# google/balloon-learning-environment

Hardware: AMD Instinct MI355X
Metric: env-steps/sec at 65 536 parallel envs; achieved HBM GB/s fraction of peak (higher is better)
Workload: dtype f32+f64

## Files before the change

balloon_learning_environment_amd/csrc/ble_step_core.h:

```cpp
#pragma once
#include "ble_physics.h"

namespace ble {

struct StateDev {
  float *x, *y, *pressure, *ambient_temperature, *internal_temperature, *envelope_volume, *superpressure, *mols_air, *battery_charge;
  float *acs_power, *acs_mass_flow, *solar_charging, *power_load;
  const float *center_lat_deg, *center_lng_deg, *upwelling_infrared, *alpha;
  const int64_t* start_unix;
  int32_t *time_elapsed_s, *sunrise_h_rel, *sunset_rel;
  uint8_t *status, *last_command, *alt_fsm, *env_fsm, *power_paused;
  double* episode_cache;
};
struct EnvRegs {
  float x, y, p, t_amb, t_int, vol, sp, n_air, batt;
  float acs_power, mdot, charge, load;
  int32_t t_elapsed, sunrise_h, sunset;
  uint8_t status, alt_fsm, env_fsm, paused;
};
struct EnvConst {
  float lat0_deg, lng0_deg, ir, alpha;
  int64_t start_unix;
};
struct EnvHoisted {
  AtmBase atm;
  double sin_lat0, cos_lat0;
  double q_earth;
  uint32_t flags;
};
constexpr int kEpisodeCacheRows = 7;
BLE_FN EnvHoisted hoist_constants(const EnvConst& c) {
  EnvHoisted h;
  h.atm = atm_base((double)c.alpha);
  sincos_f64((double)c.lat0_deg * (kPiD / 180.0), &h.sin_lat0, &h.cos_lat0);
  h.flags = 0;
  h.q_earth = earth_heat_per_area_f64((double)c.ir, &h.flags);
  return h;
}
BLE_FN uint32_t float_bits(float v) { uint32_t u; __builtin_memcpy(&u, &v, 4); return u; }
BLE_FN void episode_cache_keys(const EnvConst& c, uint64_t* k1, uint64_t* k2) {
  *k1 = ((uint64_t)float_bits(c.alpha) << 32) | (uint64_t)float_bits(c.lat0_deg);
  *k2 = ((uint64_t)float_bits(c.ir) << 32) | 0x80000000ull;
}
BLE_FN void episode_cache_store(double* cache, int64_t n, int64_t i, const EnvConst& c, const EnvHoisted& h) {
  uint64_t k1, k2;
  episode_cache_keys(c, &k1, &k2);
  k2 |= (uint64_t)(h.flags & 0x7fffffffu);
  double d1, d2;
  __builtin_memcpy(&d1, &k1, 8); __builtin_memcpy(&d2, &k2, 8);
  cache[i] = h.atm.p1; cache[n + i] = h.atm.p2; cache[2 * n + i] = h.sin_lat0; cache[3 * n + i] = h.cos_lat0;
  cache[4 * n + i] = h.q_earth; cache[5 * n + i] = d1; cache[6 * n + i] = d2;
}
struct EpisodeCacheRow { double v[kEpisodeCacheRows]; };
BLE_FN EpisodeCacheRow episode_cache_load(const double* cache, int64_t n, int64_t i) {
  EpisodeCacheRow r;
#pragma unroll
  for (int k = 0; k < kEpisodeCacheRows; ++k) r.v[k] = cache[k * n + i];
  return r;
}
BLE_FN bool episode_cache_hit(const EpisodeCacheRow& r, const EnvConst& c) {
  uint64_t k1, k2, g1, g2;
  episode_cache_keys(c, &k1, &k2);
  __builtin_memcpy(&g1, &r.v[5], 8); __builtin_memcpy(&g2, &r.v[6], 8);
  return g1 == k1 && (g2 & 0xffffffff80000000ull) == k2;
}
BLE_FN EnvHoisted hoisted_from_cache(const EpisodeCacheRow& r, const EnvConst& c) {
  EnvHoisted h;
  atm_base_linear((double)c.alpha, &h.atm);
  h.atm.p1 = r.v[0]; h.atm.p2 = r.v[1];
  h.sin_lat0 = r.v[2]; h.cos_lat0 = r.v[3]; h.q_earth = r.v[4];
  uint64_t g2;
  __builtin_memcpy(&g2, &r.v[6], 8);
  h.flags = (uint32_t)(g2 & 0x7fffffffull);
  return h;
}


BLE_FN double inv_cbrt_volume(double vol) {
  double yc = (double)f_exp2((-1.0f / 3.0f) * f_log2((float)vol));
  return yc * d_fma(-vol * yc, yc * yc, 4.0) * (1.0 / 3.0);
}
BLE_FN double d_min_raw(double a, double b) {
#if defined(__HIP_DEVICE_COMPILE__)
  double r; asm("v_min_f64 %0, %1, %2" : "=v"(r) : "v"(a), "v"(b)); return r;
#else
  return d_min(a, b);
#endif
}
BLE_FN double d_max_raw(double a, double b) {
#if defined(__HIP_DEVICE_COMPILE__)
  double r; asm("v_max_f64 %0, %1, %2" : "=v"(r) : "v"(a), "v"(b)); return r;
#else
  return d_max(a, b);
#endif
}
struct LayerCursor {
  int lay;
  double lapse_cur;
  double kl_cur;
  double cur_hi, cur_lo;
};
BLE_FN double stride_pressure(const AtmWindow& win, const LayerCursor& lc, double p, double rp, double vol, double n_air,
                              double t_amb, double t_at_p, double yc, const StrideK& K, double drag_arg = VehicleDefault::drag_arg) {
  const double mass = d_fma(kAirMolarMassD, n_air, K.dry_mass);
  const double num = d_fma(p * vol, K.m_over_r, -mass * t_amb);
  const double dir = __builtin_copysign(1.0, num);
  const double arg = drag_arg * __builtin_fabs(num) * rp * (yc * yc);
  const double rate = atm_rate_over_delta_height_f64(win, lc.lay, lc.lapse_cur, lc.kl_cur, lc.cur_hi, lc.cur_lo, p, rp, dir, t_at_p,
                                                     d_max(arg, 1e-30), K);
  return d_fma(rate, K.ten, p);
}
BLE_FN double stride_internal_temperature(double vol, double yc, double t_int, double t_amb, double p, float flux, float att,
                                          double q_earth, const StrideK& K, double thermal_scale = VehicleDefault::thermal_scale) {
  return t_int + thermal_increment_f64(vol, yc, t_int, t_amb, p, (double)((flux * att) * (0.25f * kSolarAbsorptivityTotal)), q_earth, K, thermal_scale);
}
template <bool kNodeFromTable = true>
BLE_FN void stride_acs(const double* acs_poly, int eff, double sp, double p, double rp, double t_int, float* acs_w, double* mdot_d,
                       const StrideK& K, double valve_k = VehicleDefault::valve_k) {
  const double a2 = d_max((2.0 * (kAirMolarMassD / kGasConstantD)) * (sp * (sp + p)), 1e-30);
  const double mdot_up = (valve_k * a2) * d_rsqrt(a2 * t_int);
  const double prm1 = d_max(sp * rp, 0.0);
  double w_down, mdot_down;
  acs_down_poly<kNodeFromTable>(acs_poly, prm1, &w_down, &mdot_down, K);
  *acs_w = eff == kDown ? (float)w_down : 0.0f;
  *mdot_d = eff == kUp ? mdot_up : (eff == kDown ? mdot_down : 0.0);
}
BLE_FN double stride_mols_air(double n_air, double mdot_d) {
  return d_max(d_fma(mdot_d, 10.0 / kAirMolarMassD, n_air), 0.0);
}
BLE_FN void stride_power_from_factor(bool is_day, float panel_factor, float att, float acs_w, float* charge, float* load, float* batt,
                                     float day_load = VehicleDefault::day_load, float night_load = VehicleDefault::night_load,
                                     float capacity = VehicleDefault::capacity) {
  *charge = is_day ? solar_power_from_factor(panel_factor, att) : 0.0f;
  *load = (is_day ? day_load : night_load) + acs_w;
  *batt = f_clamp(f_fma(*charge - *load, kStride / 3600.0f, *batt), 0.0f, capacity);
}
BLE_FN void stride_power(const SunState& sun, float att, float acs_w, float* charge, float* load, float* batt,
                         float day_load = VehicleDefault::day_load, float night_load = VehicleDefault::night_load,
                         float capacity = VehicleDefault::capacity) {
  stride_power_from_factor(sun.day, solar_panel_factor(sun), att, acs_w, charge, load, batt, day_load, night_load, capacity);
}
BLE_FN double stride_ambient_advance(const AtmWindow& win, LayerCursor& lc, double p, double rp, double t_at_p, double p_new,
                                     const StrideK& K) {
  const double kInf = (double)__builtin_huge_valf();
  double anchor_p = p, anchor_rp = rp, anchor_t = t_at_p;
  const bool crossed = p_new > lc.cur_hi || !(p_new > lc.cur_lo);
  if (__builtin_expect(wave_any(crossed), 0)) if (crossed) {
    BLE_STEP_EVENT(1);
    const int lay_new = atm_window_layer(win, p_new);
    const bool low_pair = (lc.lay + lay_new) < 0;
    anchor_p = low_pair ? win.pb : win.pt;
    anchor_rp = low_pair ? win.r_pb : win.r_pt;
    anchor_t = low_pair ? win.tb : win.tt;
    lc.lay = lay_new;
    lc.lapse_cur = pick3(lay_new, win.lapse_m1, win.lapse_0, win.lapse_p1);
    lc.kl_cur = (-kAirSpecificGasD / 9.80665) * lc.lapse_cur;
    lc.cur_hi = lay_new < 0 ? kInf : (lay_new == 0 ? win.pb : win.pt);
    lc.cur_lo = lay_new < 0 ? win.pb : (lay_new == 0 ? win.pt : -kInf);
  }
  return atm_temperature_advance(anchor_t, anchor_p, anchor_rp, p_new, lc.kl_cur, K);
}

struct SolarNodes {
  double sb0, cb0, sb1, cb1, sb2, cb2;
  double sd0, cd0, hsd, hcd;
};
BLE_FN SolarNodes solar_nodes_time(const Ephemeris& e0, int64_t t0, float lng0_deg, float step_s) {
  SolarNodes n;
  double sod;
  if (__builtin_expect(t0 >= 0 && t0 < 4294967296LL, 1)) sod = (double)((uint32_t)t0 % 86400u);
  else { int64_t m = t0 % 86400; sod = (double)(m < 0 ? m + 86400 : m); }
  const double b0 = sod * (1.0 / 240.0) + 0.25 * e0.eot_min + (double)lng0_deg;
  const double half_db = 0.5 * ((double)step_s * (1.0 / 240.0) + 0.25 * (double)(e0.eot_min_rate * step_s));
  double sb0, cb0;
  sincos_f64(b0 * (kPiD / 180.0), &sb0, &cb0);
  const double hr = half_db * (kPiD / 180.0), h2 = hr * hr;
  const double sh = hr * d_fma(h2, d_fma(h2, d_fma(h2, -1.0 / 5040.0, 1.0 / 120.0), -1.0 / 6.0), 1.0);
  const double ch = d_fma(h2, d_fma(h2, d_fma(h2, -1.0 / 720.0, 1.0 / 24.0), -0.5), 1.0);
  const double sb1 = sb0 * ch + cb0 * sh, cb1 = cb0 * ch - sb0 * sh;
  const double sb2 = sb1 * ch + cb1 * sh, cb2 = cb1 * ch - sb1 * sh;
  n.sb0 = sb0; n.cb0 = cb0; n.sb1 = sb1; n.cb1 = cb1; n.sb2 = sb2; n.cb2 = cb2;
  const double sd0 = (double)e0.sin_decl, cd0 = d_sqrt_fast(d_fma(-sd0, sd0, 1.0));
  const double hsd = 0.5 * (double)(e0.sin_decl_rate * step_s), hcd = -(sd0 * d_rcp(cd0)) * hsd;
  n.sd0 = sd0; n.cd0 = cd0; n.hsd = hsd; n.hcd = hcd;
  return n;
}
template <int j>
BLE_FN double solar_node(const SolarNodes& n, double sl0, double cl0, float x_m, float y_m, float u, float v, int substeps) {
  const double x0 = (double)x_m, y0 = (double)y_m;
  const double dx = (double)u * (5.0 * (double)substeps), dy = (double)v * (5.0 * (double)substeps);
  if (j == 0) return sun_one_minus_sin_f64(sl0, cl0, x0, y0, n.sb0, n.cb0, n.sd0, n.cd0);
  if (j == 1) return sun_one_minus_sin_f64(sl0, cl0, x0 + dx, y0 + dy, n.sb1, n.cb1, n.sd0 + n.hsd, n.cd0 + n.hcd);
  return sun_one_minus_sin_f64(sl0, cl0, x0 + 2.0 * dx, y0 + 2.0 * dy, n.sb2, n.cb2, n.sd0 + 2.0 * n.hsd, n.cd0 + 2.0 * n.hcd);
}
struct SunQuadratic { float c0, c1, c2; SunThresholds thr; };
BLE_FN SunQuadratic solar_node_coefs(double f0, double f1, double f2, int substeps) {
  const double inv_2m = d_rcp((double)substeps);
  SunQuadratic sq;
  sq.c0 = (float)f0;
  sq.c1 = (float)((-f2 + 4.0 * f1 - 3.0 * f0) * inv_2m);
  sq.c2 = (float)((f2 - 2.0 * f1 + f0) * (2.0 * (inv_2m * inv_2m)));
  sq.thr = sun_thresholds(f0, substeps);
  return sq;
}
BLE_FN SunQuadratic solar_nodes_site(const SolarNodes& n, double sl0, double cl0, float x_m, float y_m, float u, float v, int substeps) {
  const double f0 = solar_node<0>(n, sl0, cl0, x_m, y_m, u, v, substeps);
  const double f1 = solar_node<1>(n, sl0, cl0, x_m, y_m, u, v, substeps);
  const double f2 = solar_node<2>(n, sl0, cl0, x_m, y_m, u, v, substeps);
  return solar_node_coefs(f0, f1, f2, substeps);
}
BLE_FN SunState sun_at_stride(int kk, const SunQuadratic& sq, const EnvConst& c, float u, float v, float x_start,
                              float y_start, int32_t t_start) {
  const float fkk = (float)kk;
  bool near;
  const float q = fkk * f_fma(fkk, sq.c2, sq.c1);
  SunState r = sun_fast(sq.c0 + q, q, sq.thr, &near);
  if (__builtin_expect(wave_any(near), 0)) if (near) {
    BLE_STEP_EVENT(0);
    kk = i_opaque(kk);
    const double dk = 10.0 * (double)kk;
    r = sun_exact((double)c.lat0_deg, (double)c.lng0_deg, d_fma(dk, (double)u, (double)x_start), d_fma(dk, (double)v, (double)y_start),
                  c.start_unix + (int64_t)(t_start + 10 * kk));
  }
  return r;
}
BLE_FN bool battery_above_99_percent(float batt, double capacity_wh = VehicleDefault::capacity_d) {
  return capacity_wh == 3058.56 ? batt >= 3027.9746f : (double)batt / capacity_wh > 0.99;
}
template <typename PowerFn>
BLE_FN float step_reward_from_power(int action, float x, float y, float batt, float acs_power, PowerFn power_end,
                                    float day_load = VehicleDefault::day_load, double capacity_wh = VehicleDefault::capacity_d) {
  float r = reward_distance(x, y);
  if (action == kDown) {
    const float pw = power_end();
    const bool excess = (pw > day_load) && battery_above_99_percent(batt, capacity_wh);
    if (!excess) {
      const float scale = f_clamp((acs_power - 100.0f) * (1.0f / 200.0f), 0.0f, 1.0f);
      r *= f_fma(-0.3f, scale, 0.95f);
    }
  }
  return r;
}
template <typename SunFn>
BLE_FN float step_reward(int action, float x, float y, float p, float batt, float acs_power, SunFn sun_end,
                         float day_load = VehicleDefault::day_load, double capacity_wh = VehicleDefault::capacity_d) {
  return step_reward_from_power(action, x, y, batt, acs_power, [&]() {
    const SunState sun = sun_end();
    return solar_power(sun, solar_attenuation(sun.sin_el, p, sun.day));
  }, day_load, capacity_wh);
}

constexpr int kTermSaveRows = 14, kTermSaveStride = 64;
constexpr int kTermAbsBit = 1 << 16;
struct NoHelper { static constexpr bool kOn = false; };
struct SunRecord { float diff, panel_factor, flux; uint32_t bits; };
template <class V = VehicleDefault, class H = NoHelper>
BLE_FN int agent_step(EnvRegs& s, const EnvConst& c, const EnvHoisted& hc, int action, const WindCorners& corners, const WindQuery& wq,
                      float noise_u, float noise_v, int substeps, const double* acs_poly, const StrideK& K, float* term_save,
                      float* reward, uint32_t* flags, const V& veh = V(), H* helper = nullptr) {
  BLE_STEP_TICK(0);
  float u, v;
  if constexpr (H::kOn) {
    wind_blend_corners(corners, wq, &u, &v);
    u += noise_u; v += noise_v;
    helper->publish(s.x, s.y, u, v, s.t_elapsed);
  }
  const float p0_in = s.p;
  double p = (double)s.p;
  const AtmWindow win = atm_window_from(hc.atm, (double)c.alpha, p, flags);
  double altitude, t_at_p;
  atm_at_pressure_f64(win, (double)c.alpha, p, &altitude, &t_at_p);
  LayerCursor lc;
  lc.lay = 0; lc.lapse_cur = win.lapse_0; lc.kl_cur = (-kAirSpecificGasD / 9.80665) * win.lapse_0; lc.cur_hi = win.pb; lc.cur_lo = win.pt;

  int eff = action;
  if (veh.power_layer)
    eff = power_safety(action, s.t_elapsed, s.batt, &s.sunrise_h, &s.sunset, &s.paused, veh.night_load_d, veh.capacity_d);
  eff = envelope_safety(eff, s.sp, &s.env_fsm, veh.max_sp);
  eff = altitude_safety(eff, altitude, &s.alt_fsm);
  BLE_STEP_TICK(1);

  const int64_t t0 = c.start_unix + (int64_t)s.t_elapsed;
  const Ephemeris e0 = ephemeris(t0);
  const float step_s = (float)(10 * substeps);
  const float fl0 = e0.flux, dfl = e0.flux_rate * 10.0f;
  BLE_STEP_TICK(2);
  if constexpr (!H::kOn) {
    wind_blend_corners(corners, wq, &u, &v);
    u += noise_u; v += noise_v;
  }
  BLE_STEP_TICK(3);
  const SolarNodes nodes = solar_nodes_time(e0, t0, c.lng0_deg, step_s);
  const SunQuadratic sq = solar_nodes_site(nodes, hc.sin_lat0, hc.cos_lat0, s.x, s.y, u, v, substeps);
  BLE_STEP_TICK(4);
  const float x_start = s.x, y_start = s.y;
  const int32_t t_start = s.t_elapsed;
  auto sun_at = [&](int kk) -> SunState {
    return sun_at_stride(kk, sq, c, u, v, x_start, y_start, t_start);
  };
  const double q_earth = hc.q_earth;
  *flags |= hc.flags;

  double t_amb = (double)s.t_amb, t_int = (double)s.t_int, n_air = (double)s.n_air, vol = (double)s.vol,
         sp = (double)s.sp;
  double t_int_lo = t_int, t_int_hi = t_int;
  float x = s.x, y = s.y, batt = s.batt;
  float acs_w = s.acs_power, charge = s.charge, load = s.load;
  double mdot_d = (double)s.mdot;
  int status = kOk;

  float* const term_word = term_save + (kTermSaveRows - 1) * kTermSaveStride;
  *term_word = 0.0f;
  auto stride = [&](const int k) __attribute__((always_inline)) {
    const float pf = (float)p;
    const double rp = d_rcp(p);
    t_int_lo = d_min_raw(t_int_lo, t_int); t_int_hi = d_max_raw(t_int_hi, t_int);
    SunState sun;
    SunRecord rec;
    float flux;
    if constexpr (!H::kOn) {
      const float fk = (float)k;
      sun = sun_at(k);
      flux = f_fma(fk, dfl, fl0);
    } else {
      rec = helper->record(k);
      flux = rec.flux;
    }

    const double yc = inv_cbrt_volume(vol);
    const double p_new = stride_pressure(win, lc, p, rp, vol, n_air, t_amb, t_at_p, yc, K, veh.drag_arg);

    float att;
    if constexpr (!H::kOn) att = solar_attenuation(sun.sin_el, pf, sun.day);
    else att = solar_attenuation_from_diff(rec.diff, pf, (rec.bits & 1u) != 0);
    const double t_int_new = stride_internal_temperature(vol, yc, t_int, t_amb, p, flux, att, q_earth, K, veh.thermal_scale);

    double vol_new, sp_new;
    superpressure_volume_f64(n_air, t_int, p, rp, &vol_new, &sp_new, K, veh.dvdp, veh.four_dvdp, veh.inv_dvdp);
    bool terminal = !(sp_new <= veh.max_sp) || sp_new <= 0.0;

    stride_acs(acs_poly, eff, sp, p, rp, t_int, &acs_w, &mdot_d, K, veh.valve_k);
    const double n_air_new = stride_mols_air(n_air, mdot_d);

    if constexpr (!H::kOn) stride_power(sun, att, acs_w, &charge, &load, &batt, veh.day_load, veh.night_load, veh.capacity);
    else stride_power_from_factor((rec.bits & 1u) != 0, rec.panel_factor, att, acs_w, &charge, &load, &batt, veh.day_load, veh.night_load, veh.capacity);
    terminal = terminal || batt <= 0.0f;

    x = f_fma(u, kStride, x);
    y = f_fma(v, kStride, y);
    t_amb = t_at_p;
    t_at_p = stride_ambient_advance(win, lc, p, rp, t_at_p, p_new, K);
    p = p_new; t_int = t_int_new; vol = vol_new; sp = sp_new; n_air = n_air_new;
    if (__builtin_expect(wave_any(terminal), 0)) if (terminal && __builtin_bit_cast(int, *term_word) == 0) {
      int st = kOk;
      if (!(sp <= veh.max_sp)) st = kBurst;
      if (sp <= 0.0) st = kZeroPressure;
      if (batt <= 0.0f) st = kOutOfPower;
      const float parked[kTermSaveRows - 1] = {x, y, (float)p, (float)t_amb, (float)t_int, (float)vol, (float)sp, (float)n_air, batt,
                                               acs_w, (float)mdot_d, charge, load};
#pragma unroll
      for (int j = 0; j < kTermSaveRows - 1; ++j) term_save[j * kTermSaveStride] = parked[j];
      const int strides = i_opaque(k + 1);
      const int abs_bad = absorptivity_out_of_range(t_int_lo) || absorptivity_out_of_range(t_int_hi) ? kTermAbsBit : 0;
      *term_word = __builtin_bit_cast(float, st | (strides << 8) | abs_bad);
      if constexpr (H::kOn) helper->park_reward_record(k + 1);
    }
  };
  int ks = 0;
#pragma unroll 1
  for (; ks + 1 < substeps; ks += 2) { stride(ks); stride(ks + 1); }
  if (ks < substeps) stride(ks);
  BLE_STEP_TICK(5);
  s.x = x; s.y = y; s.p = (float)p; s.t_amb = (float)t_amb; s.t_int = (float)t_int; s.vol = (float)vol;
  s.sp = (float)sp; s.n_air = (float)n_air; s.batt = batt;
  s.acs_power = acs_w; s.mdot = (float)mdot_d; s.charge = charge; s.load = load;
  int k = substeps;
  const int word = __builtin_bit_cast(int, *term_word);
  const bool done = word != 0;
  SunRecord rec_end;
  if constexpr (H::kOn) rec_end = helper->record_end(substeps);
  bool abs_bad = absorptivity_out_of_range(t_int_lo) || absorptivity_out_of_range(t_int_hi);
  if (__builtin_expect(wave_any(done), 0)) if (done) {
    s.x = term_save[0]; s.y = term_save[kTermSaveStride]; s.p = term_save[2 * kTermSaveStride]; s.t_amb = term_save[3 * kTermSaveStride];
    s.t_int = term_save[4 * kTermSaveStride]; s.vol = term_save[5 * kTermSaveStride]; s.sp = term_save[6 * kTermSaveStride];
    s.n_air = term_save[7 * kTermSaveStride]; s.batt = term_save[8 * kTermSaveStride]; s.acs_power = term_save[9 * kTermSaveStride];
    s.mdot = term_save[10 * kTermSaveStride]; s.charge = term_save[11 * kTermSaveStride]; s.load = term_save[12 * kTermSaveStride];
    status = word & 0xff; k = (word >> 8) & 0xff; abs_bad = (word & kTermAbsBit) != 0;
    if constexpr (H::kOn) rec_end = helper->parked_reward_record();
  }
  s.t_elapsed += 10 * k;
  s.status = (uint8_t)status;
  *flags |= abs_bad ? kFlagAbsorptivity : 0u;

  *flags |= (s.p > 101325.0f || s.p < 0.0f || p0_in > 101325.0f || p0_in < 0.0f) ? kFlagSolarRange : 0u;

  if constexpr (!H::kOn) {
  *reward = step_reward(action, s.x, s.y, s.p, s.batt, s.acs_power, [&]() { return sun_at(k); }, veh.day_load, veh.capacity_d);
  } else {
    *reward = step_reward_from_power(action, s.x, s.y, s.batt, s.acs_power, [&]() {
      return solar_power_from_factor(rec_end.panel_factor, solar_attenuation_from_diff(rec_end.diff, s.p, (rec_end.bits & 1u) != 0));
    }, veh.day_load, veh.capacity_d);
  }
  BLE_STEP_TICK(6);
  return eff;
}

}
```

balloon_learning_environment_amd/csrc/ble_step_helper.h:

```cpp
#pragma once
#include "ble_step_core.h"

namespace ble {

constexpr int kHelperGroups = 4;
constexpr int kHelperBlock = 2 * 64 * kHelperGroups;
constexpr int kHelperRing = 32;

struct alignas(16) HelperGroupShared {
  SunRecord ring[kHelperRing][64];
  SunRecord reward_park[64];
  float x[64], y[64], u[64], v[64];
  int32_t t_elapsed[64];
  unsigned long long live;
  int steps_published;
  int records_taken;
  int records_ready;
  int pad_;
};
struct HelperShared {
  HelperGroupShared group[kHelperGroups];
  int ticket[4];
  int placed[kHelperBlock / 64];
};

BLE_FN int helper_uniform(int v) { return __builtin_amdgcn_readfirstlane(v); }
BLE_FN int helper_counter_load(const int* p) { return helper_uniform(__hip_atomic_load(p, __ATOMIC_RELAXED, __HIP_MEMORY_SCOPE_WORKGROUP)); }
BLE_FN void helper_counter_store(int* p, int v) {
  asm volatile("s_waitcnt lgkmcnt(0)" ::: "memory");
  __hip_atomic_store(p, v, __ATOMIC_RELAXED, __HIP_MEMORY_SCOPE_WORKGROUP);
}
BLE_FN void helper_wait_above(const int* p, int need, int* seen) {
  int r = helper_counter_load(p);
  while (r <= need) { __builtin_amdgcn_s_sleep(1); r = helper_counter_load(p); }
  *seen = r;
  asm volatile("" ::: "memory");
}

BLE_FN int helper_assign_roles(HelperShared& sh, int hw_wave, int lane) {
  const int simd = (int)__builtin_amdgcn_s_getreg((1 << 11) | (4 << 6) | 4) & 3;
  const int tid = hw_wave * 64 + lane;
  if (tid < 4) sh.ticket[tid] = 0;
  if (tid < kHelperGroups) {
    sh.group[tid].live = 0ull; sh.group[tid].steps_published = 0; sh.group[tid].records_taken = 0; sh.group[tid].records_ready = 0;
  }
  __syncthreads();
  if (lane == 0) {
    const int t = atomicAdd(&sh.ticket[simd], 1);
    sh.placed[hw_wave] = t < 2 ? 2 * simd + t : -1;
  }
  __syncthreads();
  constexpr int kWaves = kHelperBlock / 64;
  int taken = 0, unplaced_before = 0;
#pragma unroll
  for (int q = 0; q < kWaves; ++q) {
    const int p = helper_uniform(sh.placed[q]);
    if (p >= 0) taken |= 1 << p;
    else if (q < hw_wave) ++unplaced_before;
  }
  int role = helper_uniform(sh.placed[hw_wave]);
  if (role < 0) {
    role = 0;
#pragma unroll
    for (int r = 0, free_seen = 0; r < kWaves; ++r)
      if (!((taken >> r) & 1)) { if (free_seen == unplaced_before) role = r; ++free_seen; }
  }
  return role;
}

struct HelperMain {
  static constexpr bool kOn = true;
  HelperGroupShared* g;
  int lane;
  int base, ready_seen, steps_done;
  BLE_FN void publish(float x, float y, float u, float v, int32_t t_elapsed) {
    g->x[lane] = x; g->y[lane] = y; g->u[lane] = u; g->v[lane] = v; g->t_elapsed[lane] = t_elapsed;
    g->live = __builtin_amdgcn_ballot_w64(true);
    helper_counter_store(&g->steps_published, steps_done);
  }
  BLE_FN SunRecord read(int index) const { return g->ring[index & (kHelperRing - 1)][lane]; }
  BLE_FN SunRecord record(int k) {
    const int index = helper_uniform(base) + k;
    if ((k & 1) == 0) {
      asm volatile("" ::: "memory");
      __hip_atomic_store(&g->records_taken, index, __ATOMIC_RELAXED, __HIP_MEMORY_SCOPE_WORKGROUP);
    }
    if (__builtin_expect(helper_uniform(ready_seen) <= index, 0)) helper_wait_above(&g->records_ready, index, &ready_seen);
    return read(index);
  }
  BLE_FN SunRecord record_end(int substeps) {
    const int index = helper_uniform(base) + substeps;
    if (__builtin_expect(helper_uniform(ready_seen) <= index, 0)) helper_wait_above(&g->records_ready, index, &ready_seen);
    const SunRecord r = read(index);
    base = index + 1;
    return r;
  }
  BLE_FN void park_reward_record(int k) {
    const int index = helper_uniform(base) + k;
    int seen;
    helper_wait_above(&g->records_ready, index, &seen);
    g->reward_park[lane] = read(index);
  }
  BLE_FN SunRecord parked_reward_record() const { return g->reward_park[lane]; }
  BLE_FN void publish_idle() {
    g->live = 0ull;
    helper_counter_store(&g->steps_published, steps_done);
  }
};

BLE_FN void helper_wave(const StateDev& st, HelperGroupShared* g, int lane, int64_t i, bool in_range, int substeps, int n_steps) {
  EnvConst c = {0.0f, 0.0f, 0.0f, 0.0f, 0};
  int32_t t_s = 0;
  bool ok = false;
  if (in_range) {
    c.lat0_deg = st.center_lat_deg[i]; c.lng0_deg = st.center_lng_deg[i];
    c.ir = st.upwelling_infrared[i]; c.alpha = st.alpha[i]; c.start_unix = st.start_unix[i];
    t_s = st.time_elapsed_s[i];
    ok = st.status[i] == kOk;
  }
  double sin_lat0 = 0.0, cos_lat0 = 1.0;
  if (ok) sincos_f64((double)c.lat0_deg * (kPiD / 180.0), &sin_lat0, &cos_lat0);
  const float step_s = (float)(10 * substeps);
  int next = 0;
  int taken_seen = 0, published_seen = 0;
  bool all_frozen = false;
#pragma unroll 1
  for (int step = 0; step < n_steps; ++step) {
    int64_t t0 = c.start_unix + (int64_t)t_s;
    Ephemeris e0 = {};
    SolarNodes nodes = {};
    if (!all_frozen) {
      e0 = ephemeris(t0);
      nodes = solar_nodes_time(e0, t0, c.lng0_deg, step_s);
    }
    if (published_seen <= step) helper_wait_above(&g->steps_published, step, &published_seen);
    const unsigned long long live_mask = g->live;
    const uint32_t live_lo = (uint32_t)helper_uniform((int)(uint32_t)live_mask), live_hi = (uint32_t)helper_uniform((int)(uint32_t)(live_mask >> 32));
    if (live_lo == 0u && live_hi == 0u) { all_frozen = true; continue; }
    const bool live = (((lane < 32 ? live_lo : live_hi) >> (lane & 31)) & 1u) != 0u;
    float x = g->x[lane], y = g->y[lane], u = g->u[lane], v = g->v[lane];
    int32_t t_pub = g->t_elapsed[lane];
    if (!live) { x = 0.0f; y = 0.0f; u = 0.0f; v = 0.0f; t_pub = t_s; }
    const bool moved = t_pub != t_s;
    if (__builtin_expect(wave_any(moved), 0)) if (moved) {
      t_s = t_pub;
      t0 = c.start_unix + (int64_t)t_s;
      e0 = ephemeris(t0);
      nodes = solar_nodes_time(e0, t0, c.lng0_deg, step_s);
    }
    const float fl0 = e0.flux, dfl = e0.flux_rate * 10.0f;
    const SunQuadratic sq = solar_nodes_site(nodes, sin_lat0, cos_lat0, x, y, u, v, substeps);
#pragma unroll 1
    for (int kk = 0; kk <= substeps; ++kk) {
      const SunState sun = sun_at_stride(kk, sq, c, u, v, x, y, t_s);
      SunRecord rec;
      rec.diff = solar_airmass_diff(sun.sin_el);
      rec.panel_factor = solar_panel_factor(sun);
      rec.flux = f_fma((float)kk, dfl, fl0);
      rec.bits = sun.day ? 1u : 0u;
      if (__builtin_expect(next - taken_seen >= kHelperRing, 0)) helper_wait_above(&g->records_taken, next - kHelperRing, &taken_seen);
      g->ring[next & (kHelperRing - 1)][lane] = rec;
      ++next;
      helper_counter_store(&g->records_ready, next);
    }
    t_s += 10 * substeps;
  }
}

}
```

profiles/isa_histogram.py:

```python
import os
import re
import subprocess
import sys
import tempfile

sys.path.insert(0, os.path.dirname(os.path.abspath(__file__)))
from isa_compare import ROOT, assemble

DEFAULT_KERNEL = 'ble_step_kernelILb0EN3ble14VehicleDefaultEEE'
CLASSES = ['fp64 arithmetic', 'fp32 arithmetic', 'v_cmp*', 'v_cndmask*', 'v_cvt*', 'other vector', 'moves', 'LDS', 'memory', 'SALU',
           'branches', 'waits', 's_nop']


def classify(op: str) -> str:
  if op.startswith('v_cmp'):
    return 'v_cmp*'
  if op.startswith('v_cndmask'):
    return 'v_cndmask*'
  if op.startswith('v_cvt'):
    return 'v_cvt*'
  if op.startswith(('v_mov', 'v_accvgpr', 'v_readfirstlane', 'v_readlane', 'v_writelane', 'v_swap')):
    return 'moves'
  if op.startswith('v_'):
    if '_f64' in op:
      return 'fp64 arithmetic'
    if '_f32' in op or '_f16' in op:
      return 'fp32 arithmetic'
    return 'other vector'
  if op.startswith('ds_'):
    return 'LDS'
  if op.startswith(('global_', 'buffer_', 'flat_', 'scratch_', 's_load', 's_buffer_load')):
    return 'memory'
  if op.startswith('s_waitcnt') or op.startswith('s_wait'):
    return 'waits'
  if op == 's_nop':
    return 's_nop'
  if op.startswith(('s_cbranch', 's_branch')):
    return 'branches'
  return 'SALU'


def kernel_body(asm: str, key: str):
  lines = asm.splitlines()
  start = next(i for i, l in enumerate(lines) if re.match(r'^\S*' + re.escape(key) + r'\S*:', l))
  out, parents, loop = [], {}, None
  for i in range(start + 1, len(lines)):
    if re.match(r'^\.Lfunc_end\d+:', lines[i]):
      break
    text, _, comment = lines[i].partition(';')
    text = text.strip()
    label = re.match(r'^(\.LBB\d+_\d+):', text)
    if label or re.match(r'^\s*; %bb\.\d+:', lines[i]):
      block_comment = lines[i]
      for j in range(i + 1, min(i + 4, len(lines))):
        if not lines[j].lstrip().startswith(';') or '%bb.' in lines[j]:
          break
        block_comment += lines[j]
      m = re.search(r'in Loop: Header=(BB\d+_\d+)', block_comment)
      if m:
        loop = '.L' + m.group(1)
      elif 'Loop Header' in block_comment and label:
        loop = label.group(1)
        m = re.findall(r'Parent Loop (BB\d+_\d+)', block_comment)
        parents[loop] = '.L' + m[-1] if m else None
      else:
        loop = None
    if text and (label or not text.startswith('.')):
      out.append((i + 1, text, loop))
  return lines[start].split(':')[0], out, parents


def in_loop(loop, header, parents) -> bool:
  while loop is not None:
    if loop == header:
      return True
    loop = parents.get(loop)
  return False


def hot_path(body, parents, header, inner=None):
  label_at = {t[:-1]: k for k, (_, t, _) in enumerate(body) if t.endswith(':')}
  k, path, seen, after_inner = label_at[header], [], set(), False
  while True:
    if k in seen:
      return path
    seen.add(k)
    _, t, loop = body[k]
    if inner and t == inner + ':':
      k = next(label_at[m.group(1)] for j in range(k, len(body)) if body[j][2] == inner
               for m in [re.match(r'^s_cbranch\S*\s+(\.LBB\d+_\d+)', body[j][1])] if m and not in_loop(body[label_at[m.group(1)]][2], inner, parents))
      after_inner = True
      continue
    if not t.endswith(':'):
      path.append(k)
      m = re.match(r'^s_(c?)branch\S*\s+(\.LBB\d+_\d+)', t)
      if m:
        target = label_at[m.group(2)]
        if m.group(2) == header:
          return path
        if m.group(1) == '':
          k = target
          continue
        if after_inner and t.startswith('s_cbranch_scc'):
          after_inner = False
          k = target
          continue
        over_inner = inner is not None and k < label_at[inner] < target
        if target > k and not over_inner and in_loop(body[target][2], header, parents) and not re.match(r'^s_branch\b', body[target - 1][1]):
          k = target
          continue
    k += 1


SEEDS_F64 = ('v_rcp_f64', 'v_rsq_f64', 'v_sqrt_f64')
TRANS_F32 = ('v_exp_f32', 'v_log_f32', 'v_rcp_f32', 'v_rsq_f32', 'v_sqrt_f32', 'v_sin_f32', 'v_cos_f32', 'v_rcp_iflag_f32')
COST_ROWS = ['fp64 seeds', 'fp32 transcendentals', 'conversions to / from fp64', 'other fp64', 'other vector', 'not on the VALU pipe']
COST_NS = {'fp64 seeds': (7.0, 6.85), 'fp32 transcendentals': (4.15, 3.5), 'conversions to / from fp64': (3.1, 1.6), 'other fp64': (2.1, 2.05),
           'other vector': (2.1, 1.05), 'not on the VALU pipe': (2.1, 0.0)}


def cost_class(op: str) -> str:
  base = op.split('_e32')[0].split('_e64')[0].split('_sdwa')[0].split('_dpp')[0]
  if base in SEEDS_F64:
    return 'fp64 seeds'
  if base in TRANS_F32:
    return 'fp32 transcendentals'
  if op.startswith('v_cvt') and 'f64' in op:
    return 'conversions to / from fp64'
  if op.startswith('v_'):
    return 'other fp64' if ('_f64' in op or '_b64' in op) else 'other vector'
  return 'not on the VALU pipe'


def cost(body, path):
  rows = {r: [0, 0.0, 0.0] for r in COST_ROWS}
  for k in path:
    r = cost_class(body[k][1].split()[0])
    rows[r][0] += 1; rows[r][1] += COST_NS[r][0]; rows[r][2] += COST_NS[r][1]
  return rows, sum(v[1] for v in rows.values()), sum(v[2] for v in rows.values())


def report_cost(title, body, stride_path, strides_per_iteration, step_path):
  rs, s1, s2 = cost(body, stride_path)
  rp, p1, p2 = cost(body, step_path)
  d = float(strides_per_iteration)
  print(f'{title}: cost-weighted hot path (ns; `valu_op_cost` of r02_microbench.md)')
  print('| Class | Per stride: count | one wave | two waves | Per-step part: count | one wave | two waves |')
  print('|---|---|---|---|---|---|---|')
  for r in COST_ROWS:
    print(f'| {r} | {rs[r][0] / d:g} | {rs[r][1] / d:.1f} | {rs[r][2] / d:.1f} | {rp[r][0]} | {rp[r][1]:.1f} | {rp[r][2]:.1f} |')
  print(f'| **all** | {len(stride_path) / d:g} | {s1 / d:.1f} | {s2 / d:.1f} | {len(step_path)} | {p1:.1f} | {p2:.1f} |')
  step1, step2 = 18 * s1 / d + p1, 18 * s2 / d + p2
  print(f'per agent step (18 strides + the per-step part): one wave {step1 / 1e3:.2f} us, two waves (pipe time) {step2 / 1e3:.2f} us')
  print()
  return step1, step2


def histogram(body, path):
  h = dict.fromkeys(CLASSES, 0)
  for k in path:
    h[classify(body[k][1].split()[0])] += 1
  return h


def analyse(asm: str, key: str):
  name, body, parents = kernel_body(asm, key)
  f64 = {}
  for _, t, loop in body:
    if loop and '_f64' in t.split()[0]:
      f64[loop] = f64.get(loop, 0) + 1
  size = {}
  for _, t, loop in body:
    if loop and not t.endswith(':'):
      size[loop] = size.get(loop, 0) + 1
  def innermost(l):
    return all(size.get(c, 0) < 30 and c not in f64 for c, p in parents.items() if p == l)
  def hot_f64(l):
    return sum('_f64' in body[k][1].split()[0] for k in hot_path(body, parents, l))
  stride = max((l for l in f64 if innermost(l)), key=hot_f64)
  step = parents[stride]
  return name, body, hot_path(body, parents, stride), hot_path(body, parents, step, inner=stride)


def analyse_helper_role(body, parents, main_step):
  size = {}
  for _, t, loop in body:
    if loop and not t.endswith(':'):
      size[loop] = size.get(loop, 0) + 1
  def root(l):
    while parents.get(l) is not None:
      l = parents[l]
    return l
  total = {}
  for l, v in size.items():
    if root(l) != root(main_step):
      total[root(l)] = total.get(root(l), 0) + v
  if not total:
    return None
  step = max(total, key=total.get)
  inner = [l for l in size if l != step and in_loop(l, step, parents)]
  if not inner:
    return None
  record = max(inner, key=size.get)
  return hot_path(body, parents, record), hot_path(body, parents, step, inner=record)


def report_helper_role(body, record_path, step_path, with_cost=False):
  hr, hp = histogram(body, record_path), histogram(body, step_path)
  print(f'helper wave: record loop .s lines {body[record_path[0]][0]}-{body[record_path[-1]][0]} (one record = one stride per iteration)')
  print('| Class | Per record (stride) | Per-step part |')
  print('|---|---|---|')
  for c in CLASSES:
    print(f'| {c} | {hr[c]} | {hp[c]} |')
  print(f'| **all** | {len(record_path)} | {len(step_path)} |')
  vec = lambda h: sum(v for c, v in h.items() if c in CLASSES[:9])
  print(f'vector (incl. LDS, memory) / scalar per record: {vec(hr)} / {len(record_path) - vec(hr)}; per-step part: {vec(hp)} / {len(step_path) - vec(hp)}')
  print()
  return report_cost('helper wave', body, record_path, 1, step_path) if with_cost else None


def report(rev: str, asm: str, key: str, dump: bool, with_cost: bool = False) -> None:
  name, body, stride_path, step_path = analyse(asm, key)
  hs, hp = histogram(body, stride_path), histogram(body, step_path)
  print(f'## {rev}: {name[:90]}')
  print(f'stride loop: .s lines {body[stride_path[0]][0]}-{body[stride_path[-1]][0]}; the per-step part is scattered over {len({body[k][2] for k in step_path})} loop levels of .s lines {min(body[k][0] for k in step_path)}-{max(body[k][0] for k in step_path)}')
  print('| Class | Per two strides | Per stride | Per-step part |')
  print('|---|---|---|---|')
  for c in CLASSES:
    print(f'| {c} | {hs[c]} | {hs[c] / 2:g} | {hp[c]} |')
  print(f'| **all** | {len(stride_path)} | {len(stride_path) / 2:g} | {len(step_path)} |')
  vec = lambda h: sum(v for c, v in h.items() if c in CLASSES[:9])
  print(f'vector (incl. LDS, memory) / scalar per two strides: {vec(hs)} / {len(stride_path) - vec(hs)}; per-step part: {vec(hp)} / {len(step_path) - vec(hp)}')
  print()
  main_cost = report_cost('main wave', body, stride_path, 2, step_path) if with_cost else None
  _, _, parents = kernel_body(asm, key)
  helper = analyse_helper_role(body, parents, body[step_path[0]][2] if body[step_path[0]][2] else None) if 'helper' in name else None
  if helper:
    helper_cost = report_helper_role(body, *helper, with_cost=with_cost)
    if with_cost:
      print(f'both waves, pipe time per agent step (two-waves column, main + helper): {(main_cost[1] + helper_cost[1]) / 1e3:.2f} us')
      print()
    if dump == 'helper':
      for k in helper[0]:
        print(f'{body[k][0]:7d}  {classify(body[k][1].split()[0]):16s} {body[k][1]}')
  if dump:
    for k in (step_path if dump == 'step' else stride_path):
      print(f'{body[k][0]:7d}  {classify(body[k][1].split()[0]):16s} {body[k][1]}')


def main() -> int:
  args = sys.argv[1:]
  dump = 'step' if '--dump-step' in args else ('helper' if '--dump-helper' in args else '--dump' in args)
  key = DEFAULT_KERNEL
  if '--kernel' in args:
    key = args[args.index('--kernel') + 1]
    del args[args.index('--kernel'):args.index('--kernel') + 2]
  with_cost = '--cost' in args
  revs = [a for a in args if not a.startswith('--')] or ['tree']
  with tempfile.TemporaryDirectory() as tmp:
    for rev in revs:
      tree = ROOT
      if rev.endswith('.s'):
        report(rev, open(rev).read(), key, dump, with_cost)
        continue
      if rev != 'tree':
        tree = os.path.join(tmp, re.sub(r'\W', '_', rev))
        os.makedirs(tree)
        archive = subprocess.check_output(['git', '-C', ROOT, 'archive', rev, 'balloon_learning_environment_amd/csrc', 'include'])
        subprocess.run(['tar', 'x', '-C', tree], input=archive, check=True)
      out = os.path.join(tempfile.gettempdir(), 'isa_histogram_' + re.sub(r'\W', '_', rev) + '.s')
      report(rev, assemble(tree, out), key, dump, with_cost)
  return 0


if __name__ == '__main__':
  sys.exit(main())
```

Before: 4.849 billion.

## Compact lit lanes in helper wave and distribute sun strides as work items

The helper wave no longer evaluates every stride on every lane. Lanes whose site is provably dark for the whole step are detected up front, and their ring slots are filled with zero records. The strides of the lit lanes are flattened into (lane, stride) items that are spread across all 64 lanes, with per-site coefficients pulled in via ds_bpermute. A cost model falls back to the per-lane loop when compaction would not pay. This removes divergent idle work for night lanes, at the cost of extra permute traffic, more complex ring synchronisation, and a margin-based darkness test that has to stay conservative.

Result: no change. 4.858 billion (median of 3 runs) (+0.2%).

```diff
diff --git a/balloon_learning_environment_amd/csrc/ble_step_core.h b/balloon_learning_environment_amd/csrc/ble_step_core.h
--- a/balloon_learning_environment_amd/csrc/ble_step_core.h
+++ b/balloon_learning_environment_amd/csrc/ble_step_core.h
@@ -209,18 +209,24 @@
   const double f2 = solar_node<2>(n, sl0, cl0, x_m, y_m, u, v, substeps);
   return solar_node_coefs(f0, f1, f2, substeps);
 }
+BLE_FN SunState sun_stride_fast(int kk, const SunQuadratic& sq, bool* near) {
+  const float fkk = (float)kk;
+  const float q = fkk * f_fma(fkk, sq.c2, sq.c1);
+  return sun_fast(sq.c0 + q, q, sq.thr, near);
+}
+BLE_FN SunState sun_stride_exact(int kk, const EnvConst& c, float u, float v, float x_start, float y_start, int32_t t_start) {
+  const double dk = 10.0 * (double)kk;
+  return sun_exact((double)c.lat0_deg, (double)c.lng0_deg, d_fma(dk, (double)u, (double)x_start), d_fma(dk, (double)v, (double)y_start),
+                   c.start_unix + (int64_t)(t_start + 10 * kk));
+}
 BLE_FN SunState sun_at_stride(int kk, const SunQuadratic& sq, const EnvConst& c, float u, float v, float x_start,
                               float y_start, int32_t t_start) {
-  const float fkk = (float)kk;
   bool near;
-  const float q = fkk * f_fma(fkk, sq.c2, sq.c1);
-  SunState r = sun_fast(sq.c0 + q, q, sq.thr, &near);
+  SunState r = sun_stride_fast(kk, sq, &near);
   if (__builtin_expect(wave_any(near), 0)) if (near) {
     BLE_STEP_EVENT(0);
     kk = i_opaque(kk);
-    const double dk = 10.0 * (double)kk;
-    r = sun_exact((double)c.lat0_deg, (double)c.lng0_deg, d_fma(dk, (double)u, (double)x_start), d_fma(dk, (double)v, (double)y_start),
-                  c.start_unix + (int64_t)(t_start + 10 * kk));
+    r = sun_stride_exact(kk, c, u, v, x_start, y_start, t_start);
   }
   return r;
 }
diff --git a/balloon_learning_environment_amd/csrc/ble_step_helper.h b/balloon_learning_environment_amd/csrc/ble_step_helper.h
--- a/balloon_learning_environment_amd/csrc/ble_step_helper.h
+++ b/balloon_learning_environment_amd/csrc/ble_step_helper.h
@@ -1,5 +1,6 @@
 #pragma once
 #include "ble_step_core.h"
+#include "ble_step_items.h"
 
 namespace ble {
 
@@ -108,6 +109,29 @@
   }
 };
 
+BLE_FN SunRecord helper_record(const SunState& sun, int kk, float fl0, float dfl) {
+  SunRecord rec;
+  rec.diff = solar_airmass_diff(sun.sin_el);
+  rec.panel_factor = solar_panel_factor(sun);
+  rec.flux = f_fma((float)kk, dfl, fl0);
+  rec.bits = sun.day ? 1u : 0u;
+  return rec;
+}
+BLE_FN int helper_fetch(int src, int v) { return __builtin_amdgcn_ds_bpermute(src << 2, v); }
+BLE_FN float helper_fetch(int src, float v) { return __builtin_bit_cast(float, helper_fetch(src, __builtin_bit_cast(int, v))); }
+
+BLE_FN void helper_room(HelperGroupShared* g, int index, int* taken_seen) {
+  if (__builtin_expect(index - *taken_seen >= kHelperRing, 0)) helper_wait_above(&g->records_taken, index - kHelperRing, taken_seen);
+}
+BLE_FN void helper_fill_night(HelperGroupShared* g, int lane, bool dark, int first, int last) {
+#pragma unroll 1
+  for (int index = first; index <= last; ++index) if (dark) g->ring[index & (kHelperRing - 1)][lane] = SunRecord{0.0f, 0.0f, 0.0f, 0u};
+}
+
+constexpr int kHelperItemStrides = kHelperRing - 2;
+constexpr int kHelperItemCost = 194;
+constexpr int kHelperLaneCost = 79;
+
 BLE_FN void helper_wave(const StateDev& st, HelperGroupShared* g, int lane, int64_t i, bool in_range, int substeps, int n_steps) {
   EnvConst c = {0.0f, 0.0f, 0.0f, 0.0f, 0};
   int32_t t_s = 0;
@@ -150,19 +174,73 @@
     }
     const float fl0 = e0.flux, dfl = e0.flux_rate * 10.0f;
     const SunQuadratic sq = solar_nodes_site(nodes, sin_lat0, cos_lat0, x, y, u, v, substeps);
-#pragma unroll 1
-    for (int kk = 0; kk <= substeps; ++kk) {
-      const SunState sun = sun_at_stride(kk, sq, c, u, v, x, y, t_s);
-      SunRecord rec;
-      rec.diff = solar_airmass_diff(sun.sin_el);
-      rec.panel_factor = solar_panel_factor(sun);
-      rec.flux = f_fma((float)kk, dfl, fl0);
-      rec.bits = sun.day ? 1u : 0u;
-      if (__builtin_expect(next - taken_seen >= kHelperRing, 0)) helper_wait_above(&g->records_taken, next - kHelperRing, &taken_seen);
-      g->ring[next & (kHelperRing - 1)][lane] = rec;
-      ++next;
-      helper_counter_store(&g->records_ready, next);
-    }
+    const int base = next;
+    const int32_t t_start = t_s;
+    auto record_by_lane = [=, &taken_seen](int kk) {
+      const SunState sun = sun_at_stride(kk, sq, c, u, v, x, y, t_start);
+      helper_room(g, base + kk, &taken_seen);
+      g->ring[(base + kk) & (kHelperRing - 1)][lane] = helper_record(sun, kk, fl0, dfl);
+      helper_counter_store(&g->records_ready, base + kk + 1);
+    };
+    record_by_lane(0);
+    const bool lit = live && !helper_lane_dark(sq, substeps);
+    const unsigned long long lit_mask = __builtin_amdgcn_ballot_w64(lit);
+    const uint32_t lit_lo = (uint32_t)lit_mask, lit_hi = (uint32_t)(lit_mask >> 32);
+    const int n_lit = __builtin_popcount(lit_lo) + __builtin_popcount(lit_hi);
+    const int rank = (int)__builtin_amdgcn_mbcnt_hi(lit_hi, __builtin_amdgcn_mbcnt_lo(lit_lo, 0u));
+    const int lane_of_rank = __builtin_amdgcn_ds_permute((lit ? rank : n_lit + lane - rank) << 2, lane);
+    const bool dark = live && !lit;
+#pragma unroll 1
+    for (int k0 = 0; k0 < substeps; k0 += kHelperItemStrides) {
+      const int sc = substeps - k0 < kHelperItemStrides ? substeps - k0 : kHelperItemStrides;
+      const int n_iter = (sc * n_lit + 63) >> 6;
+      if (n_iter * kHelperItemCost >= sc * kHelperLaneCost) {
+#pragma unroll 1
+        for (int kk = k0 + 1; kk <= k0 + sc; ++kk) record_by_lane(kk);
+        continue;
+      }
+      int complete = 0;
+#pragma unroll 1
+      for (int m = 0; m < n_iter; ++m) {
+        const HelperItem it = helper_item(64 * m + lane, n_lit, sc);
+        const int done = helper_uniform(helper_strides_complete(m, n_lit, sc));
+        const int src = __builtin_amdgcn_ds_bpermute((it.valid ? it.j : 0) << 2, lane_of_rank);
+        SunQuadratic sqi;
+        sqi.c0 = helper_fetch(src, sq.c0); sqi.c1 = helper_fetch(src, sq.c1); sqi.c2 = helper_fetch(src, sq.c2);
+        sqi.thr.d_day = helper_fetch(src, sq.thr.d_day); sqi.thr.d_s33 = helper_fetch(src, sq.thr.d_s33);
+        sqi.thr.d_s27 = helper_fetch(src, sq.thr.d_s27); sqi.thr.d_r5 = helper_fetch(src, sq.thr.d_r5);
+        sqi.thr.band = sq.thr.band;
+        const float fl0_i = helper_fetch(src, fl0), dfl_i = helper_fetch(src, dfl);
+        const int kk = k0 + (it.valid ? it.k : 1);
+        bool near;
+        SunState sun = sun_stride_fast(kk, sqi, &near);
+        near = near && it.valid;
+        if (__builtin_expect(wave_any(near), 0)) {
+          EnvConst ci = {0.0f, 0.0f, 0.0f, 0.0f, 0};
+          ci.lat0_deg = helper_fetch(src, c.lat0_deg); ci.lng0_deg = helper_fetch(src, c.lng0_deg);
+          const uint32_t start_lo = (uint32_t)helper_fetch(src, (int)(uint32_t)c.start_unix);
+          const uint32_t start_hi = (uint32_t)helper_fetch(src, (int)(uint32_t)((uint64_t)c.start_unix >> 32));
+          ci.start_unix = (int64_t)(((uint64_t)start_hi << 32) | start_lo);
+          const float x_i = helper_fetch(src, x), y_i = helper_fetch(src, y), u_i = helper_fetch(src, u), v_i = helper_fetch(src, v);
+          const int32_t t_i = helper_fetch(src, t_start);
+          if (near) sun = sun_stride_exact(kk, ci, u_i, v_i, x_i, y_i, t_i);
+        }
+        const SunRecord rec = helper_record(sun, kk, fl0_i, dfl_i);
+        helper_room(g, base + k0 + (done < sc ? done + 1 : sc), &taken_seen);
+        if (it.valid) g->ring[(base + kk) & (kHelperRing - 1)][src] = rec;
+        if (done > complete) {
+          helper_fill_night(g, lane, dark, base + k0 + complete + 1, base + k0 + done);
+          complete = done;
+          helper_counter_store(&g->records_ready, base + k0 + done + 1);
+        }
+      }
+      if (complete < sc) {
+        helper_room(g, base + k0 + sc, &taken_seen);
+        helper_fill_night(g, lane, dark, base + k0 + complete + 1, base + k0 + sc);
+        helper_counter_store(&g->records_ready, base + k0 + sc + 1);
+      }
+    }
+    next = base + substeps + 1;
     t_s += 10 * substeps;
   }
 }
diff --git a/balloon_learning_environment_amd/csrc/ble_step_items.h b/balloon_learning_environment_amd/csrc/ble_step_items.h
--- /dev/null
+++ b/balloon_learning_environment_amd/csrc/ble_step_items.h
@@ -0,0 +1,30 @@
+#pragma once
+#include "ble_step_core.h"
+
+namespace ble {
+
+constexpr float kHelperDarkMargin = 1.0e-4f;
+BLE_FN bool helper_lane_dark(const SunQuadratic& sq, int substeps) {
+  const float fs = (float)substeps;
+  const float q_end = fs * f_fma(fs, sq.c2, sq.c1);
+  const float sag = (0.25f * fabsf(sq.c2)) * (fs * fs);
+  return (sq.thr.d_day + f_minnum(0.0f, q_end)) - sag > kHelperDarkMargin;
+}
+
+BLE_FN int helper_items_div(int t, int L) {
+  const float inv = 1.0f / (float)L;
+  return (int)(((float)t + 0.5f) * inv);
+}
+struct HelperItem { int k, j; bool valid; };
+BLE_FN HelperItem helper_item(int t, int L, int S) {
+  const int q = helper_items_div(t, L);
+  HelperItem it;
+  it.k = 1 + q; it.j = t - q * L; it.valid = t < S * L;
+  return it;
+}
+BLE_FN int helper_strides_complete(int m, int L, int S) {
+  const int k = helper_items_div(64 * (m + 1), L);
+  return k < S ? k : S;
+}
+
+}
diff --git a/profiles/isa_histogram.py b/profiles/isa_histogram.py
--- a/profiles/isa_histogram.py
+++ b/profiles/isa_histogram.py
@@ -78,7 +78,7 @@
   return False
 
 
-def hot_path(body, parents, header, inner=None):
+def hot_path(body, parents, header, inner=None, through_execz=False):
   label_at = {t[:-1]: k for k, (_, t, _) in enumerate(body) if t.endswith(':')}
   k, path, seen, after_inner = label_at[header], [], set(), False
   while True:
@@ -87,7 +87,7 @@
     seen.add(k)
     _, t, loop = body[k]
     if inner and t == inner + ':':
-      k = next(label_at[m.group(1)] for j in range(k, len(body)) if body[j][2] == inner
+      k = next(label_at[m.group(1)] for j in range(k, len(body)) if in_loop(body[j][2], inner, parents)
                for m in [re.match(r'^s_cbranch\S*\s+(\.LBB\d+_\d+)', body[j][1])] if m and not in_loop(body[label_at[m.group(1)]][2], inner, parents))
       after_inner = True
       continue
@@ -100,6 +100,9 @@
           return path
         if m.group(1) == '':
           k = target
+          continue
+        if through_execz and t.startswith('s_cbranch_execz'):
+          k += 1
           continue
         if after_inner and t.startswith('s_cbranch_scc'):
           after_inner = False
@@ -198,25 +201,49 @@
   if not total:
     return None
   step = max(total, key=total.get)
-  inner = [l for l in size if l != step and in_loop(l, step, parents)]
-  if not inner:
+  records = [l for l in size if l != step and in_loop(l, step, parents) and size[l] >= 60]
+  records = [l for l in records if not any(c != l and in_loop(c, l, parents) for c in records)]
+  if not records:
     return None
-  record = max(inner, key=size.get)
-  return hot_path(body, parents, record), hot_path(body, parents, step, inner=record)
-
-
-def report_helper_role(body, record_path, step_path, with_cost=False):
-  hr, hp = histogram(body, record_path), histogram(body, step_path)
-  print(f'helper wave: record loop .s lines {body[record_path[0]][0]}-{body[record_path[-1]][0]} (one record = one stride per iteration)')
-  print('| Class | Per record (stride) | Per-step part |')
-  print('|---|---|---|')
-  for c in CLASSES:
-    print(f'| {c} | {hr[c]} | {hp[c]} |')
-  print(f'| **all** | {len(record_path)} | {len(step_path)} |')
+  def below_step(l):
+    while parents.get(l) != step:
+      l = parents[l]
+    return l
+  around = {below_step(l) for l in records}
+  if len(around) != 1:
+    return None
+  return [(l, hot_path(body, parents, l, through_execz=any(body[k][1].startswith('ds_bpermute') for k in hot_path(body, parents, l)))) for l in records], hot_path(body, parents, step, inner=around.pop())
+
+
+def report_helper_role(body, record_paths, step_path, with_cost=False):
   vec = lambda h: sum(v for c, v in h.items() if c in CLASSES[:9])
-  print(f'vector (incl. LDS, memory) / scalar per record: {vec(hr)} / {len(record_path) - vec(hr)}; per-step part: {vec(hp)} / {len(step_path) - vec(hp)}')
+  hp = histogram(body, step_path)
+  for _, path in record_paths:
+    hr = histogram(body, path)
+    item = any(body[k][1].startswith('ds_bpermute') for k in path)
+    what = 'item loop' if item else 'record loop'
+    unit = 'Per iteration (64 items)' if item else 'Per record (stride)'
+    print(f'helper wave: {what} .s lines {body[path[0]][0]}-{body[path[-1]][0]} ({"one item per lane" if item else "one record = one stride"} per iteration)')
+    print(f'| Class | {unit} | Per-step part |')
+    print('|---|---|---|')
+    for c in CLASSES:
+      print(f'| {c} | {hr[c]} | {hp[c]} |')
+    print(f'| **all** | {len(path)} | {len(step_path)} |')
+    print(f'vector (incl. LDS, memory) / scalar per {"iteration" if item else "record"}: {vec(hr)} / {len(path) - vec(hr)}; per-step part: {vec(hp)} / {len(step_path) - vec(hp)}')
+    print()
+  if not with_cost:
+    return None
+  if len(record_paths) == 1:
+    return report_cost('helper wave', body, record_paths[0][1], 1, step_path)
+  for _, path in record_paths:
+    rows, one, two = cost(body, path)
+    item = any(body[k][1].startswith('ds_bpermute') for k in path)
+    print(f'helper wave, {"item loop, per iteration" if item else "record loop, per record"}: one wave {one:.1f} ns, two waves (pipe time) {two:.1f} ns; '
+          + ', '.join(f'{r} {rows[r][0]}' for r in COST_ROWS))
+  rows, one, two = cost(body, step_path)
+  print(f'helper wave, per-step part: one wave {one:.1f} ns, two waves (pipe time) {two:.1f} ns; ' + ', '.join(f'{r} {rows[r][0]}' for r in COST_ROWS))
   print()
-  return report_cost('helper wave', body, record_path, 1, step_path) if with_cost else None
+  return None
 
 
 def report(rev: str, asm: str, key: str, dump: bool, with_cost: bool = False) -> None:
@@ -237,11 +264,11 @@
   helper = analyse_helper_role(body, parents, body[step_path[0]][2] if body[step_path[0]][2] else None) if 'helper' in name else None
   if helper:
     helper_cost = report_helper_role(body, *helper, with_cost=with_cost)
-    if with_cost:
+    if with_cost and helper_cost:
       print(f'both waves, pipe time per agent step (two-waves column, main + helper): {(main_cost[1] + helper_cost[1]) / 1e3:.2f} us')
       print()
     if dump == 'helper':
-      for k in helper[0]:
+      for k in [k for _, path in helper[0] for k in path]:
         print(f'{body[k][0]:7d}  {classify(body[k][1].split()[0]):16s} {body[k][1]}')
   if dump:
     for k in (step_path if dump == 'step' else stride_path):
```
